# AolinFeng/PMP-VVC-TIP2023

Measured on AMD Instinct MI355X. Metric: CTUs/sec (luma QT+MTT inference+post-proc), higher is better.
Workload: dtype f16x3

## Files before the change

### include/pmp.h

```cpp
#ifndef PMP_H
#define PMP_H

#include <stdint.h>

#ifdef __cplusplus
extern "C" {
#endif

#define PMP_OK 0
#define PMP_E_INVALID (-1)
#define PMP_E_HIP (-2)
#define PMP_E_NOWEIGHTS (-3)
#define PMP_E_IO (-4)
#define PMP_E_NOMEM (-5)
#define PMP_E_NODEVICE (-6)
#define PMP_E_RANGE (-7)

enum { PMP_LUMA = 0, PMP_CHROMA = 1 };
enum { PMP_NET_LUMA_Q = 0, PMP_NET_LUMA_MSBD = 1, PMP_NET_CHROMA_Q = 2, PMP_NET_CHROMA_MSBD = 3 };

typedef struct pmp_ctx pmp_ctx;

typedef struct {
    const char *name;
// ... 143 lines not shown
} pmp_stem_shape;
int pmp_stem_forward_device(pmp_ctx *ctx, const pmp_stem_shape *shape, const float *d_x, const float *const d_w[3],
                            const float *const d_b[3], float *d_y);
int pmp_stem_backward_device(pmp_ctx *ctx, const pmp_stem_shape *shape, const float *d_x, const float *d_y, const float *const d_w[3],
                             const float *d_g_y, float *d_g_x , float *const d_g_w[3], float *const d_g_b[3]);

int pmp_infer_msbd(pmp_ctx *ctx, int comp, int qp, const uint8_t *block_y, const uint8_t *block_u, const uint8_t *block_v,
                   const float *qt_in, int64_t n, float *bt, float *dire);
int pmp_infer_msbd_device(pmp_ctx *ctx, int comp, int qp, const uint8_t *d_block_y, const uint8_t *d_block_u, const uint8_t *d_block_v,
                          const float *d_qt_in, int64_t n, float *d_bt, float *d_dire);

int pmp_read_depth_dump(const char *path, int frames, int height, int width, int is_chroma, uint8_t *qt8, uint8_t *bt16,
                        int8_t *dire16, int64_t *n_unknown);

int pmp_write_partition_file(const char *path, int frames, int height, int width, const uint8_t *hor,
                             const uint8_t *ver, const uint8_t *qt_u8, const int8_t *dire_i8);
int64_t pmp_format_partition_text(int frames, int height, int width, const uint8_t *hor, const uint8_t *ver,
                                  const uint8_t *qt_u8, const int8_t *dire_i8, char *buf, int64_t cap);

int64_t pmp_format_partition_rows(int width, int block_rows, const uint8_t *hor, const uint8_t *ver, const uint8_t *qt_u8,
                                  const int8_t *dire_i8, char *buf, int64_t cap, int64_t *row_section_bytes);
int64_t pmp_format_partition_rows_records(int width, int block_rows, const uint8_t *rec, char *buf, int64_t cap,
                                          int64_t *row_section_bytes);
int pmp_tile_partition_rows_records(int width, int block_rows, const uint8_t *rec, uint8_t *out_hor, uint8_t *out_ver, uint8_t *out_qt,
                                    int8_t *out_dire);

int pmp_write_partition_binary(const char *path, int frames, int height, int width, const uint8_t *hor, const uint8_t *ver,
                               const uint8_t *qt_u8, const int8_t *dire_i8);

int pmp_tile_partition_maps(int frames, int height, int width, const uint8_t *hor, const uint8_t *ver, const uint8_t *qt_u8,
                            const int8_t *dire_i8, uint8_t *out_hor, uint8_t *out_ver, uint8_t *out_qt, int8_t *out_dire);

int pmp_ktime_enable(pmp_ctx *ctx, uint32_t mask);
int pmp_ktime_classes(void);
const char *pmp_ktime_name(int cls);
int pmp_ktime_get(pmp_ctx *ctx, int cls, int64_t *launches, double *ms, double *flops);

int pmp_debug_set_conv_variant(int variant);

int pmp_debug_set_winograd(pmp_ctx *ctx, int on);

int pmp_debug_set_fusion(pmp_ctx *ctx, int on);

int pmp_debug_activation_report(pmp_ctx *ctx, int comp, int qp, int exps[5], float seg_amax[5], char *buf, int64_t cap);
int pmp_debug_set_activation_scales(pmp_ctx *ctx, int on);

int pmp_debug_set_taps(pmp_ctx *ctx, int on);
int64_t pmp_debug_get_tap(pmp_ctx *ctx, const char *name, double *out, int64_t cap, int dims[4], int *c_real);

int pmp_debug_poison_workspace(pmp_ctx *ctx, int pattern);

int64_t pmp_debug_pack_f16x3(const float *w, int cout, int cin, int k, uint16_t *out, int64_t cap, int *scale_exp);

int pmp_debug_read_weights_file(const char *path, int *net_id, int *qp, int *ntensors, int64_t *nfloats, double *checksum);

int pmp_debug_conv_bench(pmp_ctx *ctx, int n, int h, int w, int cin, int cout, int k, int iters, double *ms_f32,
                         double *ms_x6, double *max_abs_diff, double *max_abs_ref);

typedef struct pmp_rb_case {
    int n, h, w, cin, cout, k;
    int gate, pool, out_f32;
    int exp_x, exp_gate, exp_out;
} pmp_rb_case;
int pmp_debug_run_resblock(pmp_ctx *ctx, const pmp_rb_case *cs, const float *x, const float *w0, const float *w2, const float *wsc,
                           const float *gate, int *saturated, char *kernels, int64_t cap);

#ifdef __cplusplus
}
#endif
#endif
```

### pmp_vvc_tip2023_amd/_lib.py

```python
import ctypes as C
import os

_HERE = os.path.dirname(os.path.abspath(__file__))
LIB_PATH = os.path.join(_HERE, "libpmp_hip.so")
HOSTASAN_LIB_PATH = os.path.join(_HERE, "libpmp_hostasan.so")

PMP_LUMA, PMP_CHROMA = 0, 1
PMP_RECORD_BYTES = 1344
PMP_MSBT_LEAF_BUDGET = 4096
PMP_VAL_NSTATS = 20
PMP_LOSS_NTERMS = 13
PMP_MSBT_INCONSISTENT, PMP_MSBT_QT_DEEP, PMP_MSBT_BUDGET = 1, 2, 4
NET_IDS = {"Luma_Q": 0, "Luma_MSBD": 1, "Chroma_Q": 2, "Chroma_MSBD": 3}
ERRORS = {-1: "PMP_E_INVALID", -2: "PMP_E_HIP", -3: "PMP_E_NOWEIGHTS", -4: "PMP_E_IO", -5: "PMP_E_NOMEM", -6: "PMP_E_NODEVICE", -7: "PMP_E_RANGE"}


class PmpError(RuntimeError):
    def __init__(self, code, msg):
        super().__init__("%s (%d): %s" % (ERRORS.get(code, "PMP_E_?"), code, msg))
        self.code = code


class TensorDesc(C.Structure):
    _fields_ = [("name", C.c_char_p), ("ndim", C.c_int), ("shape", C.c_int * 4), ("offset", C.c_int64)]
# ... 77 lines not shown
    "pmp_postprocess_device": (_I, [_VP, _I, _VP, _VP, _VP, _I64, _VP, _VP, _VP, _VP]),
    "pmp_set_partition_params": (_I, [_VP, _I, C.POINTER(PartitionParams)]),
    "pmp_get_partition_params": (_I, [_VP, _I, C.POINTER(PartitionParams)]),
    "pmp_parse_partition_params": (_I, [C.c_char_p, C.POINTER(PartitionParams)]),
    "pmp_infer_postprocess": (_I, [_VP, _I, _I, _VP, _VP, _VP, _I64, _VP, _VP, _VP, _VP, _VP, _VP, _VP]),
    "pmp_infer_postprocess_device": (_I, [_VP, _I, _I, _VP, _VP, _VP, _I64, _VP, _VP, _VP, _VP, _VP, _VP, _VP]),
    "pmp_postprocess_records_device": (_I, [_VP, _I, _VP, _VP, _VP, _I64, _VP]),
    "pmp_infer_postprocess_records_device": (_I, [_VP, _I, _I, _VP, _VP, _VP, _I64, _VP]),
    "pmp_cut_blocks": (_I, [_VP, _VP, _VP, _VP, _I, _I, _I, _I, _VP, _VP, _VP]),
    "pmp_cut_blocks_device": (_I, [_VP, _VP, _VP, _VP, _I, _I, _I, _I, _VP, _VP, _VP]),
    "pmp_msbt_labels": (_I, [_VP, _I, _VP, _VP, _VP, _I64, _VP, _VP]),
    "pmp_msbt_labels_device": (_I, [_VP, _I, _VP, _VP, _VP, _I64, _VP, _VP]),
    "pmp_label_partition": (_I, [_VP, _I, _VP, _VP, _VP, _I64, _VP, _VP, _VP]),
    "pmp_label_partition_device": (_I, [_VP, _I, _VP, _VP, _VP, _I64, _VP, _VP, _VP]),
    "pmp_label_partition_records_device": (_I, [_VP, _I, _VP, _VP, _VP, _I64, _VP, _VP]),
    "pmp_val_stats": (_I, [_VP, _I, _VP, _VP, _VP, _VP, _VP, _VP, _I64, _VP]),
    "pmp_val_stats_device": (_I, [_VP, _I, _VP, _VP, _VP, _VP, _VP, _VP, _I64, _VP, _VP]),
    "pmp_parse_loss_params": (_I, [C.c_char_p, C.POINTER(LossParams)]),
    "pmp_train_loss": (_I, [_VP, _I, _I, C.POINTER(LossParams), _VP, _VP, _VP, _VP, _VP, _VP, _I64, _VP, _VP, _VP, _VP, _VP]),
    "pmp_train_loss_device": (_I, [_VP, _I, _I, C.POINTER(LossParams), _VP, _VP, _VP, _VP, _VP, _VP, _I64, _VP, _VP, _VP, _VP, _VP]),
    "pmp_resblock_forward": (_I, [_VP, C.POINTER(RbShape)] + [_VP] * 6),
    "pmp_resblock_forward_device": (_I, [_VP, C.POINTER(RbShape)] + [_VP] * 6),
    "pmp_resblock_backward": (_I, [_VP, C.POINTER(RbShape)] + [_VP] * 11),
    "pmp_resblock_backward_device": (_I, [_VP, C.POINTER(RbShape)] + [_VP] * 11),
    "pmp_trunk_saved_bytes": (_I64, [C.POINTER(TrunkShape)]),
    "pmp_trunk_forward_device": (_I, [_VP, C.POINTER(TrunkShape), _VP, _VP, _VP, _VP]),
    "pmp_trunk_backward_device": (_I, [_VP, C.POINTER(TrunkShape), _VP, _VP, _VP, _VP, _VP]),
    "pmp_trunk_unpack_device": (_I, [_VP, C.POINTER(TrunkShape), _VP, _I, _VP]),
    "pmp_stem_forward_device": (_I, [_VP, C.POINTER(StemShape), _VP, _VP, _VP, _VP]),
    "pmp_stem_backward_device": (_I, [_VP, C.POINTER(StemShape)] + [_VP] * 7),
    "pmp_infer_msbd": (_I, [_VP, _I, _I, _VP, _VP, _VP, _VP, _I64, _VP, _VP]),
    "pmp_infer_msbd_device": (_I, [_VP, _I, _I, _VP, _VP, _VP, _VP, _I64, _VP, _VP]),
    "pmp_read_depth_dump": (_I, [C.c_char_p, _I, _I, _I, _I, _VP, _VP, _VP, C.POINTER(_I64)]),
    "pmp_write_partition_file": (_I, [C.c_char_p, _I, _I, _I, _VP, _VP, _VP, _VP]),
    "pmp_write_partition_binary": (_I, [C.c_char_p, _I, _I, _I, _VP, _VP, _VP, _VP]),
    "pmp_tile_partition_maps": (_I, [_I, _I, _I, _VP, _VP, _VP, _VP, _VP, _VP, _VP, _VP]),
    "pmp_format_partition_text": (_I64, [_I, _I, _I, _VP, _VP, _VP, _VP, _VP, _I64]),
    "pmp_format_partition_rows": (_I64, [_I, _I, _VP, _VP, _VP, _VP, _VP, _I64, _VP]),
    "pmp_format_partition_rows_records": (_I64, [_I, _I, _VP, _VP, _I64, _VP]),
    "pmp_tile_partition_rows_records": (_I, [_I, _I, _VP, _VP, _VP, _VP, _VP]),
    "pmp_ktime_enable": (_I, [_VP, _U32]),
    "pmp_ktime_classes": (_I, []),
    "pmp_ktime_name": (C.c_char_p, [_I]),
    "pmp_ktime_get": (_I, [_VP, _I, C.POINTER(_I64), C.POINTER(C.c_double), C.POINTER(C.c_double)]),
    "pmp_debug_set_conv_variant": (_I, [_I]),
    "pmp_debug_set_winograd": (_I, [_VP, _I]),
    "pmp_debug_set_fusion": (_I, [_VP, _I]),
    "pmp_debug_set_activation_scales": (_I, [_VP, _I]),
    "pmp_debug_activation_report": (_I, [_VP, _I, _I, C.POINTER(_I), C.POINTER(C.c_float), C.c_char_p, _I64]),
    "pmp_debug_set_taps": (_I, [_VP, _I]),
    "pmp_debug_get_tap": (_I64, [_VP, C.c_char_p, _VP, _I64, C.POINTER(_I), C.POINTER(_I)]),
    "pmp_debug_poison_workspace": (_I, [_VP, _I]),
    "pmp_debug_pack_f16x3": (C.c_int64, [C.POINTER(C.c_float), _I, _I, _I, C.POINTER(C.c_uint16), C.c_int64, C.POINTER(C.c_int)]),
    "pmp_debug_conv_bench": (_I, [_VP, _I, _I, _I, _I, _I, _I, _I] + [C.POINTER(C.c_double)] * 4),
    "pmp_debug_run_resblock": (_I, [_VP, _VP] + [C.POINTER(C.c_float)] * 5 + [C.POINTER(_I), C.c_char_p, _I64]),
}

_lib = None


def open_library(path, subset=False):
    if not os.path.isfile(path):
        raise ImportError("%s is missing - build it with `make -C %s` (or __graft_entry__.build())"
                          % (path, os.path.join(_HERE, "csrc")))
    lib = C.CDLL(path)
    for name, (res, args) in SIGNATURES.items():
        if subset and not hasattr(lib, name):
            continue
        fn = getattr(lib, name)
        fn.restype = res
        fn.argtypes = args
    return lib


def _torch_first():
    import sys
    if "torch" not in sys.modules:
        try:
            import torch
        except ImportError:
            pass


def load(path=None):
    global _lib
    if _lib is None:
        _torch_first()
        _lib = open_library(path or LIB_PATH)
    elif path is not None and os.path.abspath(path) != os.path.abspath(_lib._name):
        raise RuntimeError("a different build of the library is already loaded: %s" % _lib._name)
    return _lib


def check(rc, ctx=None):
    if rc < 0:
        msg = load().pmp_last_error(ctx)
        raise PmpError(int(rc), msg.decode() if msg else "")
    return rc
```

### pmp_vvc_tip2023_amd/csrc/api_debug.cpp

```cpp
#include <algorithm>
#include <cmath>
#include <cstring>

#include "pmp_host.h"

namespace pmp {

KScope::KScope(pmp_ctx *c_, hipStream_t stream_, int cls_, double flops_) : c(c_), stream(stream_), cls(cls_), on(false), a(nullptr), b(nullptr), flops(flops_)
{
    on = (c->kmask >> cls) & 1u;
    if (on) { a = c->event_pool.get(); b = c->event_pool.get(); hipEventRecord(a, stream); }
}

KScope::~KScope()
{
    if (on) { hipEventRecord(b, stream); c->krec[cls].push_back(KTimeRec{a, b, flops}); }
}

void ktime_drain(pmp_ctx *c)
{
    for (int k = 0; k < K_NCLASS; ++k) {
        for (auto &r : c->krec[k]) {
            float ms = 0.f;
            hipEventSynchronize(r.b);
// ... 30 lines not shown
}

}

using namespace pmp;

extern "C" {

int pmp_debug_set_conv_variant(int variant)
{
    int rc;
    if (abl_set_conv_variant(variant, &rc)) return rc;
    if (variant != 2) return set_err(nullptr, PMP_E_INVALID, "pmp_debug_set_conv_variant: this library ships only the default form (2); the A/B and timing-only builds are in tools/abl/libpmp_hip_abl.so (make -C tools/abl)");
    return PMP_OK;
}

int pmp_debug_set_fusion(pmp_ctx *c, int on)
{
    CHECK_CTX(c);
    const int rc = settle(c);
    if (rc != PMP_OK) return rc;
    if (on < 0 || on > 3) return set_err(c, PMP_E_INVALID, "pmp_debug_set_fusion: 0 (none), 1 (all), 2 (16x16 tails only), 3 (32x32 ResidualBlocks only)");
    c->fuse16 = (on == 1 || on == 2) ? 1 : 0;
    c->fuse32 = (on == 1 || on == 3) ? 1 : 0;
    return PMP_OK;
}

int pmp_debug_set_winograd(pmp_ctx *c, int on)
{
    CHECK_CTX(c);
    int rc = settle(c);
    if (rc != PMP_OK) return rc;
    if (abl_set_winograd(c, on, &rc)) return rc;
    if (on) return set_err(c, PMP_E_INVALID, "pmp_debug_set_winograd: the Winograd-x form is built into tools/abl/libpmp_hip_abl.so only (make -C tools/abl)");
    return PMP_OK;
}

int pmp_debug_conv_bench(pmp_ctx *c, int n, int h, int w, int cin, int cout, int k, int iters, double *ms_f32, double *ms_x6,
                         double *max_abs_diff, double *max_abs_ref)
{
    CHECK_CTX(c);
    if (n <= 0 || (h & 15) || (w & 15) || (cin & 15) || (cout & 15) || cout > 64 || (k != 1 && k != 3 && k != 5) || iters <= 0)
        return set_err(c, PMP_E_INVALID, "pmp_debug_conv_bench: bad shape");
    const size_t nx = (size_t)n * cin * h * w, ny = (size_t)n * cout * h * w;
    std::vector<float> hx(nx), hw((size_t)cout * cin * k * k);
    unsigned long long st = 0x1234567ull;
    auto rnd = [&]() { st = st * 6364136223846793005ull + 1442695040888963407ull; return (float)((st >> 40) / 16777216.0) * 2.f - 1.f; };
    for (auto &v : hx) v = rnd() * 3.f;
    const float ws = 1.f / sqrtf((float)cin * k * k);
    for (auto &v : hw) v = rnd() * ws;
    std::vector<float> wp = pack_mfma(hw.data(), cout, cin, k, k, cout, cin);
    const bool h2 = c->precision == PMP_PRECISION_F16X3;
    const int kexp = h2_scale_exp(hw.data(), hw.size());
    std::vector<unsigned short> wx = h2 ? pack_h2(hw.data(), cout, cin, k, k, cout, cin, kexp) : pack_x6(hw.data(), cout, cin, k, k, cout, cin);
    AblBench ab;
    DevBuf bx, by, by2, bwp, bxs, bys, bwx;
    hipError_t e = hipSuccess;
    auto A = [&](DevBuf &b, size_t bytes) {
        if (e != hipSuccess) return;
        if ((e = hipMalloc(&b.p, bytes)) == hipSuccess) b.cap = bytes;
        else b.p = nullptr;
    };
    A(bx, nx * 4); A(by, ny * 4); A(by2, ny * 4); A(bwp, wp.size() * 4);
    A(bxs, nx * 6); A(bys, ny * 6); A(bwx, wx.size() * 2);
    int rc = PMP_OK;
    if (e != hipSuccess) rc = hip_fail(c, e, "hipMalloc(conv bench)");
    if (rc == PMP_OK) {
        float *dx = (float *)bx.p, *dy = (float *)by.p, *dy2 = (float *)by2.p, *dwp = (float *)bwp.p;
        unsigned short *dxs = (unsigned short *)bxs.p, *dys = (unsigned short *)bys.p, *dwx = (unsigned short *)bwx.p;
        hipMemcpy(dx, hx.data(), nx * 4, hipMemcpyHostToDevice);
        hipMemcpy(dwp, wp.data(), wp.size() * 4, hipMemcpyHostToDevice);
        hipMemcpy(dwx, wx.data(), wx.size() * 2, hipMemcpyHostToDevice);
        ConvMfmaArgs a{};
        a.x = dx; a.w = dwp; a.out = dy; a.N = n; a.H = h; a.W = w; a.Cin = cin; a.Cout = cout; a.KH = a.KW = k; a.relu = 1;
        ConvX6Args b{};
        b.x = dxs; b.x_stride = nx; b.w = dwx; b.out = dys; b.out_stride = ny;
        b.N = n; b.H = h; b.W = w; b.Cin = cin; b.Cout = cout; b.KH = b.KW = k; b.relu = 1;
        b.out_scale = std::ldexp(1.f, -kexp);
        abl_bench_prepare(c, ab, hw.data(), k, cin, cout, h2, b);
        auto launch_split = [&]() { return h2 ? launch_conv_h2(c->stream, b) : launch_conv_x6(c->stream, b); };
        hipEvent_t e0 = c->event_pool.get(), e1 = c->event_pool.get();
        if (h2) launch_f32_to_split2(c->stream, dx, dxs, nx, nx);
        else launch_f32_to_split3(c->stream, dx, dxs, nx, nx);
        launch_conv_mfma(c->stream, a);
        e = launch_split();
        float ms = 0.f;
        hipEventRecord(e0, c->stream);
        for (int i = 0; i < iters; ++i) launch_conv_mfma(c->stream, a);
        hipEventRecord(e1, c->stream); hipEventSynchronize(e1); hipEventElapsedTime(&ms, e0, e1);
        if (ms_f32) *ms_f32 = ms / iters;
        hipEventRecord(e0, c->stream);
        for (int i = 0; i < iters; ++i) launch_split();
        hipEventRecord(e1, c->stream); hipEventSynchronize(e1); hipEventElapsedTime(&ms, e0, e1);
        if (ms_x6) *ms_x6 = ms / iters;
        abl_bench_report(c, ab, h2, n, h, w, k, cout, b, launch_split);
        if (h2) launch_split2_to_f32(c->stream, dys, dy2, ny, ny);
        else launch_split3_to_f32(c->stream, dys, dy2, ny, ny);
        std::vector<float> y1(ny), y2(ny);
        hipMemcpyAsync(y1.data(), dy, ny * 4, hipMemcpyDeviceToHost, c->stream);
        hipMemcpyAsync(y2.data(), dy2, ny * 4, hipMemcpyDeviceToHost, c->stream);
        hipError_t es = hipStreamSynchronize(c->stream);
        if (e == hipSuccess) e = es;
        if (e == hipSuccess) e = hipGetLastError();
        double md = 0, mr = 0;
        for (size_t i = 0; i < ny; ++i) { md = fmax(md, fabs((double)y1[i] - y2[i])); mr = fmax(mr, fabs((double)y1[i])); }
        if (max_abs_diff) *max_abs_diff = md;
        if (max_abs_ref) *max_abs_ref = mr;
// ... 165 lines not shown
```

### pmp_vvc_tip2023_amd/csrc/conv_f16x3.hip

```cpp
#include <cstdio>
#include <type_traits>

#include "pmp_kernels.h"
#include "split3.h"

namespace pmp {

template <int KH, int KW, int NTHR = 256>
struct StagePlanH {
    unsigned off[GeoH<KH, KW, 16, NTHR>::NLD];
    unsigned valid;
};

template <int KH, int KW, int NTHR = 256>
__device__ __forceinline__ void h2_plan(StagePlanH<KH, KW, NTHR> &p, size_t plane_stride, int H, int W, int ty, int tx)
{
    typedef GeoH<KH, KW, 16, NTHR> G;
    constexpr int PY = KH / 2, PX = KW / 2;
    p.valid = 0;
#pragma unroll
    for (int k = 0; k < G::NLD; ++k) {
        const int i = min((int)threadIdx.x + k * NTHR, G::PIECES - 1);
        const int sp = i / G::PLANE, j = i - sp * G::PLANE, pix = j >> 1, half = j & 1;
        const int row = pix / G::TW, col = pix - row * G::TW;
// ... 211 lines not shown
                for (int m = 0; m < RW; ++m)
#pragma unroll
                    for (int nt = 0; nt < CW; ++nt) acc[m][nt] = __builtin_amdgcn_mfma_f32_16x16x32_f16(w0[nt], x0[m], acc[m][nt], 0, 0, 0);
                __builtin_amdgcn_sched_barrier(0);
                if (ks + 1 < NK) {
                    const char *pn = xaddr(ks + 1);
#pragma unroll
                    for (int m = 0; m < RW; ++m) x0[m] = *reinterpret_cast<const f16x8 *>(pn + m * G::TW * 32);
                }
                __builtin_amdgcn_sched_barrier(0);
#pragma unroll
                for (int m = 0; m < RW; ++m)
#pragma unroll
                    for (int nt = 0; nt < CW; ++nt) acc[m][nt] = __builtin_amdgcn_mfma_f32_16x16x32_f16(w0[nt], x1[m], acc[m][nt], 0, 0, 0);
                __builtin_amdgcn_sched_barrier(0);
                if (!W0DB) {
#pragma unroll
                    for (int nt = 0; nt < CW; ++nt) w0[nt] = wf[(0 * NT + nt) * 64];
                }
                __builtin_amdgcn_sched_barrier(0);
            }
            if (MODE == 1 && g < 2) {
                const char *pl = buf + O_LAST + pb;
#pragma unroll
                for (int m = 0; m < RW; ++m) {
                    x0[m] = *reinterpret_cast<const f16x8 *>(pl + m * G::TW * 32);
                    x1[m] = *reinterpret_cast<const f16x8 *>(pl + G::PLANE * 16 + m * G::TW * 32);
                }
            }
        }
        if (more) h2_stage_store<KH, KW, NTHR>(plan, lds + ((cb + 1) & 1) * G::BUF, rs, NK > LAG ? (NK - LAG) * PER : 0);
        __syncthreads();
    };

    typedef std::integral_constant<int, 0> M0;
    typedef std::integral_constant<int, 1> M1;
    typedef std::integral_constant<int, 2> M2;
    typedef std::integral_constant<int, 0> T0;
    typedef std::integral_constant<int, 1> T1;
    typedef std::integral_constant<int, 2> T2;
    if (paired) {
        for (int cb = 0; cb + 2 < CB; cb += 2) {
            group(M1{}, T0{}, cb);
            group(M2{}, T0{}, cb + 1);
        }
        group(M1{}, T1{}, CB - 2);
        group(M2{}, T2{}, CB - 1);
    } else {
        for (int cb = 0; cb + 1 < CB; ++cb) group(M0{}, T0{}, cb);
        group(M0{}, T2{}, CB - 1);
    }
}

template <int NT>
__device__ __forceinline__ void h2_epilogue(const ConvX6Args &a, f32x4 (&acc)[WaveTile<NT>::RW][WaveTile<NT>::CW], int n, int ty, int tx);

template <int NT>
__device__ __forceinline__ void h2_shortcut32(const ConvX6Args &a, int n, int ty, int tx, u32x4 *lds,
                                              f32x4 (&acc)[WaveTile<NT>::RW][WaveTile<NT>::CW])
{
    typedef WaveTile<NT> WT;
    constexpr int RW = WT::RW, CW = WT::CW;
    const int tid = threadIdx.x, lane = tid & 63, wave = tid >> 6, xl = lane & 15, g = lane >> 4;
    const int rh = wave % WT::RSPLIT, ch = wave / WT::RSPLIT;
    const int W = a.W;
    const size_t grp_sz = (size_t)a.H * W * 16;
    const unsigned short *base = a.x_sc + (size_t)n * 2 * grp_sz + ((size_t)(ty * 16) * W + tx * 16) * 16;
    __syncthreads();
    u32x4 r[8];
#pragma unroll
    for (int k = 0; k < 8; ++k) {
        const int i = tid + k * 256, grp = i >> 10, plane = (i >> 9) & 1, j = i & 511, px = j >> 1, half = j & 1;
        r[k] = *reinterpret_cast<const u32x4 *>(base + plane * a.sc_stride + grp * grp_sz + ((size_t)(px >> 4) * W + (px & 15)) * 16 + half * 8);
    }
    const f16x8 *wl = reinterpret_cast<const f16x8 *>(a.w_sc) + lane + ch * CW * 64;
    f16x8 w0[CW], w1[CW];
#pragma unroll
    for (int nt = 0; nt < CW; ++nt) { w0[nt] = wl[(0 * NT + nt) * 64]; w1[nt] = wl[(1 * NT + nt) * 64]; }
#pragma unroll
    for (int k = 0; k < 8; ++k) lds[tid + k * 256] = r[k];
    __syncthreads();
    const char *px = reinterpret_cast<const char *>(lds) + (g >> 1) * 16384 + ((rh * RW * 16 + xl) * 2 + (g & 1)) * 16;
#pragma unroll
    for (int h = 0; h < RW / 2; ++h) {
        f16x8 xa[2], xb[2];
#pragma unroll
        for (int m = 0; m < 2; ++m) {
            xa[m] = *reinterpret_cast<const f16x8 *>(px + (h * 2 + m) * 16 * 32);
            xb[m] = *reinterpret_cast<const f16x8 *>(px + 8192 + (h * 2 + m) * 16 * 32);
        }
#pragma unroll
        for (int m = 0; m < 2; ++m)
#pragma unroll
            for (int nt = 0; nt < CW; ++nt) acc[h * 2 + m][nt] = __builtin_amdgcn_mfma_f32_16x16x32_f16(w1[nt], xa[m], acc[h * 2 + m][nt], 0, 0, 0);
#pragma unroll
        for (int m = 0; m < 2; ++m)
#pragma unroll
            for (int nt = 0; nt < CW; ++nt) acc[h * 2 + m][nt] = __builtin_amdgcn_mfma_f32_16x16x32_f16(w0[nt], xa[m], acc[h * 2 + m][nt], 0, 0, 0);
#pragma unroll
        for (int m = 0; m < 2; ++m)
#pragma unroll
            for (int nt = 0; nt < CW; ++nt) acc[h * 2 + m][nt] = __builtin_amdgcn_mfma_f32_16x16x32_f16(w0[nt], xb[m], acc[h * 2 + m][nt], 0, 0, 0);
    }
}

template <int KH, int KW, int NT, int SC, bool LEAN = false>
__global__ __launch_bounds__(256, NT == 4 && !LEAN ? 2 : 3) void conv_h2_kernel(ConvX6Args a)
{
    typedef GeoH<KH, KW> G;
    __shared__ u32x4 lds[2 * G::BUF];
    const int tiles_x = a.W >> 4, tiles = tiles_x * (a.H >> 4);
    int bid = blockIdx.x;
    if ((gridDim.x & 7) == 0) bid = (bid & 7) * (gridDim.x >> 3) + (bid >> 3);
    const int n = bid / tiles, t = bid - n * tiles, ty = t / tiles_x, tx = t - ty * tiles_x;
    typedef WaveTile<NT> WT;
    constexpr int RW = WT::RW, CW = WT::CW;

    f32x4 acc[RW][CW];
#pragma unroll
    for (int m = 0; m < RW; ++m)
#pragma unroll
        for (int nt = 0; nt < CW; ++nt) acc[m][nt] = (f32x4){0.f, 0.f, 0.f, 0.f};

    h2_accumulate<KH, KW, NT, LEAN>(a.x, a.x_stride, a.w, a.Cin, a.H, a.W, n, ty, tx, lds, acc);
    if (SC == 2) h2_shortcut32<NT>(a, n, ty, tx, lds, acc);
    else if (SC) h2_accumulate<1, 1, NT, LEAN>(a.x_sc, a.sc_stride, a.w_sc, a.Csc, a.H, a.W, n, ty, tx, lds, acc);
    h2_epilogue<NT>(a, acc, n, ty, tx);
}

template <int NT>
__device__ __forceinline__ void h2_epilogue(const ConvX6Args &a, f32x4 (&acc)[WaveTile<NT>::RW][WaveTile<NT>::CW], int n, int ty, int tx)
{
    typedef WaveTile<NT> WT;
    constexpr int RW = WT::RW, CW = WT::CW;
    int tid = threadIdx.x;
    asm volatile("" : "+v"(tid));
    const int lane = tid & 63, wave = tid >> 6, xl = lane & 15, g = lane >> 4;
    const int rh = wave % WT::RSPLIT, ch = wave / WT::RSPLIT;
    const int H = a.H, W = a.W;
    const size_t grp = (size_t)H * W * 16;

    const float inv_scale = a.out_scale;
    const unsigned off0 = (unsigned)(((size_t)n * NT + ch * CW) * grp + ((size_t)(ty * 16 + rh * RW) * W + tx * 16 + xl) * 16 + g * 4);
    const unsigned row_el = (unsigned)W * 16;
    const unsigned off0w = off0 - (unsigned)(g * 4) + (unsigned)(8 * (g >> 1)) + (unsigned)(g & 1) * row_el;
    u32x4 ra[RW / 2][CW], rbv[RW / 2][CW];
    auto res_load = [&](int nt, int slot) __attribute__((always_inline)) {
#pragma unroll
        for (int m = 0; m < RW; m += 2) {
            const unsigned off = off0w + (unsigned)m * row_el + (unsigned)nt * (unsigned)grp;
            ra[m >> 1][slot] = __builtin_nontemporal_load(reinterpret_cast<const u32x4 *>(a.res + off));
            rbv[m >> 1][slot] = __builtin_nontemporal_load(reinterpret_cast<const u32x4 *>(a.res + off + a.res_stride));
        }
    };
    auto res_add = [&](int nt, int slot) __attribute__((always_inline)) {
#pragma unroll
        for (int m = 0; m < RW; m += 2) {
            u32x4 p = ra[m >> 1][slot], q = rbv[m >> 1][slot];
            rows16_swap(p);
            rows16_swap(q);
            acc[m][nt] = acc[m][nt] * inv_scale + h2_sum4_lo(p, q);
            acc[m + 1][nt] = acc[m + 1][nt] * inv_scale + h2_sum4_hi(p, q);
        }
    };
    if (a.res) {
#pragma unroll
        for (int nt = 0; nt < CW; ++nt) res_load(nt, nt);
#pragma unroll
        for (int nt = 0; nt < CW; ++nt) res_add(nt, nt);
    } else {
#pragma unroll
        for (int nt = 0; nt < CW; ++nt)
#pragma unroll
            for (int m = 0; m < RW; ++m) acc[m][nt] = acc[m][nt] * inv_scale;
    }
    float amax = 0.f;
#pragma unroll
    for (int nt = 0; nt < CW; ++nt) {
#pragma unroll
        for (int m = 0; m < RW; ++m) {
            const unsigned off = off0 + (unsigned)m * row_el + (unsigned)nt * (unsigned)grp;
            f32x4 v = acc[m][nt];
            if (a.relu) { v.x = fmaxf(v.x, 0.f); v.y = fmaxf(v.y, 0.f); v.z = fmaxf(v.z, 0.f); v.w = fmaxf(v.w, 0.f); }
            if (a.gate) v *= load_split2_4(a.gate + off, a.gate_stride);
            amax = sat_amax4(amax, v);
            acc[m][nt] = v;
// ... 126 lines not shown
```

### pmp_vvc_tip2023_amd/csrc/pack.cpp

```cpp
#include <algorithm>
#include <cmath>
#include <cstring>
#include <utility>

#include "pmp_hostonly.h"

namespace pmp {

std::vector<float> pack_mfma(const float *w, int cout, int cin, int kh, int kw, int cout_pad, int cin_pad)
{
    const int taps = kh * kw, CB = cin_pad / 16, NT = cout_pad / 16;
    std::vector<float> out((size_t)CB * taps * NT * 64 * 4, 0.f);
    for (int cb = 0; cb < CB; ++cb)
        for (int t = 0; t < taps; ++t)
            for (int nt = 0; nt < NT; ++nt)
                for (int l = 0; l < 64; ++l)
                    for (int j = 0; j < 4; ++j) {
                        const int co = nt * 16 + (l & 15), ci = cb * 16 + 4 * (l >> 4) + j;
                        float v = 0.f;
                        if (co < cout && ci < cin) v = w[((size_t)co * cin + ci) * taps + t];
                        out[((((size_t)cb * taps + t) * NT + nt) * 64 + l) * 4 + j] = v;
                    }
    return out;
}
// ... 72 lines not shown
                    const float r1 = v - bf16_f32(h0);
                    const unsigned short h1 = bf16_rne(r1);
                    const float r2 = r1 - bf16_f32(h1);
                    const unsigned short h2 = bf16_rne(r2);
                    const unsigned short hs[3] = {h0, h1, h2};
                    for (int sp = 0; sp < 3; ++sp) out[(((st * 3 + sp) * NT + nt) * 64 + l) * 8 + j] = hs[sp];
                }
    return out;
}

int h2_scale_exp(const float *w, size_t n)
{
    float m = 0.f;
    for (size_t i = 0; i < n; ++i) m = std::fmax(m, std::fabs(w[i]));
    if (!(m > 0.f) || !std::isfinite(m)) return 0;
    int e = 0;
    std::frexp(m, &e);
    int k = 13 - e;
    return k < -100 ? -100 : (k > 24 ? 24 : k);
}

std::vector<unsigned short> pack_h2(const float *w, int cout, int cin, int kh, int kw, int cout_pad, int cin_pad, int scale_exp)
{
    const int taps = kh * kw, CB = cin_pad / 16, NT = cout_pad / 16;
    const bool paired = (CB % 2 == 0) && (taps % 2 == 1);
    const float S = std::ldexp(1.f, scale_exp);
    struct Half { int cb, tap; };
    std::vector<std::pair<Half, Half>> steps;
    if (paired) {
        for (int cb = 0; cb < CB; ++cb) {
            if (cb & 1) steps.push_back({{cb - 1, taps - 1}, {cb, taps - 1}});
            for (int ks = 0; ks < (taps - 1) / 2; ++ks) steps.push_back({{cb, 2 * ks}, {cb, 2 * ks + 1}});
        }
    } else {
        for (int cb = 0; cb < CB; ++cb)
            for (int ks = 0; ks < (taps + 1) / 2; ++ks) steps.push_back({{cb, 2 * ks}, {cb, 2 * ks + 1}});
    }
    std::vector<unsigned short> out(steps.size() * 2 * NT * 64 * 8, 0);
    for (size_t st = 0; st < steps.size(); ++st)
        for (int nt = 0; nt < NT; ++nt) {
            unsigned short *o0 = out.data() + ((st * 2 + 0) * NT + nt) * 512, *o1 = out.data() + ((st * 2 + 1) * NT + nt) * 512;
            for (int l = 0; l < 64; ++l) {
                const int g = l >> 4;
                const Half h = (g >> 1) ? steps[st].second : steps[st].first;
                const int co = nt * 16 + (l & 15), ci0 = h.cb * 16 + 8 * (g & 1), t = h.tap;
                float v[8];
                for (int j = 0; j < 8; ++j) v[j] = (co < cout && ci0 + j < cin && t < taps) ? w[((size_t)co * cin + ci0 + j) * taps + t] * S : 0.f;
                split8(v, o0 + l * 8, o1 + l * 8);
            }
        }
    return out;
}

std::vector<unsigned short> pack_stem_h2(const float *w32, int cin, int k1, int scale_exp)
{
    const int RPS = k1 > 8 ? 3 : 5, KPP = (k1 + RPS - 1) / RPS, KS = cin * KPP;
    const float S = std::ldexp(1.f, scale_exp);
    std::vector<unsigned short> out((size_t)KS * 3 * 2 * 64 * 8, 0);
    for (int ks = 0; ks < KS; ++ks)
        for (int nt = 0; nt < 2; ++nt)
            for (int l = 0; l < 64; ++l) {
                const int g = l >> 4, co = nt * 16 + (l & 15), ci = ks / KPP, r0 = (ks % KPP) * RPS;
                float v[8];
                for (int j = 0; j < 8; ++j) {
                    const int kk = 8 * g + j, dyl = kk / k1, dx = kk % k1, dy = r0 + dyl;
                    v[j] = (dyl < RPS && dy < k1) ? w32[(((size_t)co * cin + ci) * k1 + dy) * k1 + dx] * S : 0.f;
                }
                unsigned short *o0 = out.data() + ((((size_t)ks * 3 + 0) * 2 + nt) * 64 + l) * 8, *o1 = o0 + 2 * 64 * 8, *o2 = o1 + 2 * 64 * 8;
                split8(v, o0, o1);
                float r[8];
                unsigned short dummy[8];
                for (int j = 0; j < 8; ++j) {
                    _Float16 h0, h1;
                    std::memcpy(&h0, o0 + j, 2); std::memcpy(&h1, o1 + j, 2);
                    r[j] = (v[j] - (float)h0) - (float)h1;
                }
                split8(r, o2, dummy);
            }
    return out;
}

std::vector<float> pack_plain(const float *w, int cout, int cin, int kh, int kw)
{
    const int taps = kh * kw;
    std::vector<float> out((size_t)taps * cin * cout);
    for (int t = 0; t < taps; ++t)
        for (int ci = 0; ci < cin; ++ci)
            for (int co = 0; co < cout; ++co) out[((size_t)t * cin + ci) * cout + co] = w[((size_t)co * cin + ci) * taps + t];
    return out;
}

}

using namespace pmp;
#define set_err(ctx_unused, code, msg) set_err_global((code), (msg))

extern "C" {

int64_t pmp_debug_pack_f16x3(const float *w, int cout, int cin, int k, uint16_t *out, int64_t cap, int *scale_exp)
{
    if (!w || cout <= 0 || cin <= 0 || (k != 1 && k != 3 && k != 5) || !scale_exp)
        return set_err(nullptr, PMP_E_INVALID, "pmp_debug_pack_f16x3: bad arguments");
    const int kexp = h2_scale_exp(w, (size_t)cout * cin * k * k);
    *scale_exp = kexp;
    const std::vector<unsigned short> v = pack_h2(w, cout, cin, k, k, (cout + 15) & ~15, (cin + 15) & ~15, kexp);
    if (out && (int64_t)v.size() <= cap) memcpy(out, v.data(), v.size() * sizeof(unsigned short));
    return (int64_t)v.size();
}

}
```

### pmp_vvc_tip2023_amd/csrc/pmp_hostonly.h

```cpp
#pragma once
#include <stdint.h>

#include <string>
#include <vector>

#include "../../include/pmp.h"

namespace pmp {

int set_err_global(int code, const std::string &msg);
const char *global_err();

std::vector<float> pack_mfma(const float *w, int cout, int cin, int kh, int kw, int cout_pad, int cin_pad);
std::vector<unsigned short> pack_x6(const float *w, int cout, int cin, int kh, int kw, int cout_pad, int cin_pad);
std::vector<unsigned short> pack_h2(const float *w, int cout, int cin, int kh, int kw, int cout_pad, int cin_pad, int scale_exp);
int h2_scale_exp(const float *w, size_t n);
void h2_split8(const float *v, unsigned short *h0, unsigned short *h1);
std::vector<unsigned short> pack_stem_h2(const float *w32, int cin, int k1, int scale_exp);
std::vector<float> pack_plain(const float *w, int cout, int cin, int kh, int kw);


struct WeightTensor { std::string name; int ndim = 0; int shape[4] = {0, 0, 0, 0}; long long offset = 0; };
struct WeightFile { std::string net; int qp = -1; std::vector<WeightTensor> tensors; std::vector<float> payload;
                    std::vector<int> act_exp;
                    bool have_fp = false; uint64_t act_mtt_fp = 0, act_qt_fp = 0; };
int read_pmpw(const char *path, WeightFile &wf);
constexpr int PMP_ACT_EXP_MAX = 30;
constexpr int PMP_ACT_EXP_ATT_MAX = 6;
uint64_t fingerprint_tensors(const float *blob, const pmp_tensor_desc *descs, int ndesc);
int net_id_of(const std::string &net);

bool partition_params_valid(const pmp_partition_params &p, std::string &why);

}
```

### pmp_vvc_tip2023_amd/csrc/weights_pack.cpp

```cpp
#include <algorithm>
#include <cmath>
#include <cstring>
#include <utility>

#include "pmp_host.h"

namespace pmp {

namespace {

struct Blob {
    const float *blob;
    const pmp_tensor_desc *descs;
    int ndesc;
    const pmp_tensor_desc *find(const std::string &name) const
    {
        for (int i = 0; i < ndesc; ++i)
            if (descs[i].name && name == descs[i].name) return &descs[i];
        return nullptr;
    }
};

int roundup16(int v) { return (v + 15) & ~15; }

// ... 27 lines not shown
        fixups.clear();
        stage.clear();
        return PMP_OK;
    }
};

}

namespace {

int need(pmp_ctx *c, const Blob &b, const std::string &name, std::initializer_list<int> shape, const float **out)
{
    const pmp_tensor_desc *d = b.find(name);
    if (!d) return set_err(c, PMP_E_INVALID, "weights: missing tensor " + name);
    if (d->ndim != (int)shape.size()) return set_err(c, PMP_E_INVALID, "weights: wrong rank for " + name);
    int i = 0;
    for (int s : shape)
        if (d->shape[i++] != s) return set_err(c, PMP_E_INVALID, "weights: wrong shape for " + name);
    *out = b.blob + d->offset;
    return PMP_OK;
}

int load_rb(pmp_ctx *c, const Blob &b, Uploader &up, const std::string &name, int cin, int cout, int k, bool direct, unsigned mask)
{
    RBWeights &r = up.nw->rb[name];
    r.cin = cin; r.cout = cout; r.k = k; r.direct = direct; r.has_sc = cin != cout;
    r.cin_pad = roundup16(cin); r.cout_pad = roundup16(cout);
    const float *w0, *w2, *wsc = nullptr;
    int rc;
    if ((rc = need(c, b, name + ".left.0.weight", {cout, cin, k, k}, &w0))) return rc;
    if ((rc = need(c, b, name + ".left.2.weight", {cout, cout, k, k}, &w2))) return rc;
    if (cin != cout && (rc = need(c, b, name + ".shortcut.0.weight", {cout, cin, 1, 1}, &wsc))) return rc;
    if (direct) {
        if (!r.w0) {
            if ((rc = up.upload(pack_plain(w0, cout, cin, k, k), &r.w0))) return rc;
            if ((rc = up.upload(pack_plain(w2, cout, cout, k, k), &r.w2))) return rc;
            if (wsc && (rc = up.upload(pack_plain(wsc, cout, cin, 1, 1), &r.wsc))) return rc;
        }
    } else {
        if ((mask & (1u << PMP_PRECISION_F32)) && !r.w0) {
            if ((rc = up.upload(pack_mfma(w0, cout, cin, k, k, r.cout_pad, r.cin_pad), &r.w0))) return rc;
            if ((rc = up.upload(pack_mfma(w2, cout, cout, k, k, r.cout_pad, r.cout_pad), &r.w2))) return rc;
            if (wsc && (rc = up.upload(pack_mfma(wsc, cout, cin, 1, 1, r.cout_pad, r.cin_pad), &r.wsc))) return rc;
        }
        if ((mask & (1u << PMP_PRECISION_BF16X6)) && !r.w0x) {
            if ((rc = up.upload16(pack_x6(w0, cout, cin, k, k, r.cout_pad, r.cin_pad), &r.w0x))) return rc;
            if ((rc = up.upload16(pack_x6(w2, cout, cout, k, k, r.cout_pad, r.cout_pad), &r.w2x))) return rc;
            if (wsc && (rc = up.upload16(pack_x6(wsc, cout, cin, 1, 1, r.cout_pad, r.cin_pad), &r.wscx))) return rc;
        }
        if ((mask & (1u << PMP_PRECISION_F16X3)) && !r.w0h) {
            r.k0 = h2_scale_exp(w0, (size_t)cout * cin * k * k);
            r.k2 = h2_scale_exp(w2, (size_t)cout * cout * k * k);
            if (wsc) r.k2 = std::min(r.k2, h2_scale_exp(wsc, (size_t)cout * cin));
            if ((rc = up.upload16(pack_h2(w0, cout, cin, k, k, r.cout_pad, r.cin_pad, r.k0), &r.w0h))) return rc;
            if ((rc = up.upload16(pack_h2(w2, cout, cout, k, k, r.cout_pad, r.cout_pad, r.k2), &r.w2h))) return rc;
            if (wsc && (rc = up.upload16(pack_h2(wsc, cout, cin, 1, 1, r.cout_pad, r.cin_pad, r.k2), &r.wsch))) return rc;
        }
        if ((rc = abl_pack_rb(w0, w2, k, cin, cout, mask, r, [&](const std::vector<unsigned short> &v, unsigned short **dst) { return up.upload16(v, dst); }))) return rc;
    }
    return PMP_OK;
}

int load_head(pmp_ctx *c, const Blob &b, Uploader &up, const std::string &name, int cout, int slot)
{
    const float *w, *bias;
    int rc;
    if ((rc = need(c, b, name + ".weight", {cout, 8, 3, 3}, &w))) return rc;
    if ((rc = need(c, b, name + ".bias", {cout}, &bias))) return rc;
    if (up.nw->head_w[slot]) return PMP_OK;
    if ((rc = up.upload(pack_plain(w, cout, 8, 3, 3), &up.nw->head_w[slot]))) return rc;
    return up.upload(std::vector<float>(bias, bias + cout), &up.nw->head_b[slot]);
}

}

int load_single_rb(pmp_ctx *c, NetWeights &nw, int cin, int cout, int k, const float *w0, const float *w2, const float *wsc, unsigned mask)
{
    std::vector<float> blob(w0, w0 + (size_t)cout * cin * k * k);
    blob.insert(blob.end(), w2, w2 + (size_t)cout * cout * k * k);
    if (cin != cout) blob.insert(blob.end(), wsc, wsc + (size_t)cout * cin);
    const pmp_tensor_desc descs[3] = {{"rb.left.0.weight", 4, {cout, cin, k, k}, 0},
                                      {"rb.left.2.weight", 4, {cout, cout, k, k}, (int64_t)cout * cin * k * k},
                                      {"rb.shortcut.0.weight", 4, {cout, cin, 1, 1}, (int64_t)cout * cin * k * k + (int64_t)cout * cout * k * k}};
    Uploader up{c, &nw};
    int rc = load_rb(c, Blob{blob.data(), descs, cin != cout ? 3 : 2}, up, "rb", cin, cout, k, false, mask);
    if (rc != PMP_OK) { up.abandon(); return rc; }
    return up.finalize();
}

void free_net_weights(NetWeights &w)
{
    for (void *p : w.allocs) hipFree(p);
    w = NetWeights();
}

static int build_net(pmp_ctx *c, int net_id, const Blob &b, NetWeights &nw, unsigned mask)
{
    const bool luma = net_id == PMP_NET_LUMA_Q || net_id == PMP_NET_LUMA_MSBD;
    const bool msbd = net_id == PMP_NET_LUMA_MSBD || net_id == PMP_NET_CHROMA_MSBD;
    Uploader up{c, &nw};
    int rc = PMP_OK;
    const bool want_h2 = mask & (1u << PMP_PRECISION_F16X3);
    auto fail = [&](int code) { up.abandon(); return code; };

    if (!msbd) {
        const int cin = luma ? 1 : 3, k1 = luma ? 9 : 5, kq = luma ? 5 : 3;
        const float *w, *bias;
        if ((rc = need(c, b, "conv_q1.weight", {32, cin, k1, k1}, &w))) return fail(rc);
// ... 158 lines not shown
```

Measured before the change: 15240.

## Add sliding-window 5x5 f16x3 conv kernel with pass-paired weight packing

Adds a specialised 5x5, 64-output-channel f16x3 convolution path. Each wave slides down 20 input rows and reuses every loaded input vector across the five kernel rows, issuing MFMAs into 16 row accumulators. Weights are repacked so each pass pairs two kx taps, or the kx=4 taps of two channel blocks, with next-pass weights prefetched and the next channel group's global-to-LDS staging spread across the MFMA stream. In exchange the kernel is much more complex, uses a different accumulator tile shape and launch bound, and needs a matching host-side weight packer.

```diff
diff --git a/include/pmp.h b/include/pmp.h
--- a/include/pmp.h
+++ b/include/pmp.h
@@ -219,6 +219,8 @@
 
 int64_t pmp_debug_pack_f16x3(const float *w, int cout, int cin, int k, uint16_t *out, int64_t cap, int *scale_exp);
 
+int64_t pmp_debug_pack_f16x3_slide5(const float *w, int cout, int cin, int scale_exp, uint16_t *out, int64_t cap);
+
 int pmp_debug_read_weights_file(const char *path, int *net_id, int *qp, int *ntensors, int64_t *nfloats, double *checksum);
 
 int pmp_debug_conv_bench(pmp_ctx *ctx, int n, int h, int w, int cin, int cout, int k, int iters, double *ms_f32,
diff --git a/pmp_vvc_tip2023_amd/_lib.py b/pmp_vvc_tip2023_amd/_lib.py
--- a/pmp_vvc_tip2023_amd/_lib.py
+++ b/pmp_vvc_tip2023_amd/_lib.py
@@ -153,6 +153,7 @@
     "pmp_debug_get_tap": (_I64, [_VP, C.c_char_p, _VP, _I64, C.POINTER(_I), C.POINTER(_I)]),
     "pmp_debug_poison_workspace": (_I, [_VP, _I]),
     "pmp_debug_pack_f16x3": (C.c_int64, [C.POINTER(C.c_float), _I, _I, _I, C.POINTER(C.c_uint16), C.c_int64, C.POINTER(C.c_int)]),
+    "pmp_debug_pack_f16x3_slide5": (C.c_int64, [C.POINTER(C.c_float), _I, _I, _I, C.POINTER(C.c_uint16), C.c_int64]),
     "pmp_debug_conv_bench": (_I, [_VP, _I, _I, _I, _I, _I, _I, _I] + [C.POINTER(C.c_double)] * 4),
     "pmp_debug_run_resblock": (_I, [_VP, _VP] + [C.POINTER(C.c_float)] * 5 + [C.POINTER(_I), C.c_char_p, _I64]),
 }
@@ -187,7 +188,7 @@
     global _lib
     if _lib is None:
         _torch_first()
-        _lib = open_library(path or LIB_PATH)
+        _lib = open_library(path or LIB_PATH, subset=path is not None and os.path.abspath(path) != os.path.abspath(LIB_PATH))
     elif path is not None and os.path.abspath(path) != os.path.abspath(_lib._name):
         raise RuntimeError("a different build of the library is already loaded: %s" % _lib._name)
     return _lib
diff --git a/pmp_vvc_tip2023_amd/csrc/api_debug.cpp b/pmp_vvc_tip2023_amd/csrc/api_debug.cpp
--- a/pmp_vvc_tip2023_amd/csrc/api_debug.cpp
+++ b/pmp_vvc_tip2023_amd/csrc/api_debug.cpp
@@ -106,7 +106,7 @@
     std::vector<float> wp = pack_mfma(hw.data(), cout, cin, k, k, cout, cin);
     const bool h2 = c->precision == PMP_PRECISION_F16X3;
     const int kexp = h2_scale_exp(hw.data(), hw.size());
-    std::vector<unsigned short> wx = h2 ? pack_h2(hw.data(), cout, cin, k, k, cout, cin, kexp) : pack_x6(hw.data(), cout, cin, k, k, cout, cin);
+    std::vector<unsigned short> wx = h2 ? pack_h2_conv(hw.data(), cout, cin, k, k, cout, cin, kexp, 0) : pack_x6(hw.data(), cout, cin, k, k, cout, cin);
     AblBench ab;
     DevBuf bx, by, by2, bwp, bxs, bys, bwx;
     hipError_t e = hipSuccess;
diff --git a/pmp_vvc_tip2023_amd/csrc/conv_f16x3.hip b/pmp_vvc_tip2023_amd/csrc/conv_f16x3.hip
--- a/pmp_vvc_tip2023_amd/csrc/conv_f16x3.hip
+++ b/pmp_vvc_tip2023_amd/csrc/conv_f16x3.hip
@@ -287,14 +287,136 @@
     }
 }
 
-template <int NT>
-__device__ __forceinline__ void h2_epilogue(const ConvX6Args &a, f32x4 (&acc)[WaveTile<NT>::RW][WaveTile<NT>::CW], int n, int ty, int tx);
-
-template <int NT>
+template <int LD0, int LDS_, int ST0, int STS_, bool FETCH_>
+struct SlideSched {
+    static constexpr int ld0 = LD0, lds = LDS_, st0 = ST0, sts = STS_;
+    static constexpr bool FETCH = FETCH_;
+};
+
+__device__ __forceinline__ void h2_slide5(const unsigned short *__restrict__ x, size_t plane_stride, const unsigned short *__restrict__ wpk,
+                                          int C, int H, int W, int n, int ty, int tx, u32x4 *lds, f32x4 (&acc)[16][1])
+{
+    constexpr int NTHR = 256;
+    typedef GeoH<5, 5, 16, NTHR> G;
+    const int lane = threadIdx.x & 63, wave = threadIdx.x >> 6, xl = lane & 15, g = lane >> 4;
+    const int CB = C >> 4;
+    const size_t grp_sz = (size_t)H * W * 16;
+    const unsigned short *grp0 = x + (size_t)n * CB * grp_sz;
+    constexpr int PASS = 5 * 2 * 4 * 64;
+    const int last = (CB >> 1) * 5 + (CB & 1) * 3 - 1;
+    const f16x8 *wl = reinterpret_cast<const f16x8 *>(wpk) + lane + wave * 64;
+    f16x8 w0[5], w1[5], w0n[5], w1n[5];
+    u32x4 r[G::NLD];
+    StagePlanH<5, 5, NTHR> plan;
+    h2_plan<5, 5, NTHR>(plan, plane_stride, H, W, ty, tx);
+#pragma unroll
+    for (int ky = 0; ky < 5; ++ky) { w0[ky] = wl[(ky * 2 + 0) * 256]; w1[ky] = wl[(ky * 2 + 1) * 256]; }
+    __syncthreads();
+    h2_stage_load<5, 5, NTHR>(plan, grp0, r);
+    h2_stage_store<5, 5, NTHR>(plan, lds, r);
+    __syncthreads();
+    const int pb = (xl * 2 + (g & 1)) * 16 + (g >> 1) * 32;
+    int stream = 0;
+
+    auto pass = [&](auto t0_tag, auto sched_tag, const char *px, const unsigned short *nxt_grp, u32x4 *dst) __attribute__((always_inline)) {
+        constexpr int T0 = decltype(t0_tag)::value;
+        typedef decltype(sched_tag) S;
+        ++stream;
+        const f16x8 *wf = wl + (size_t)min(stream, last) * PASS;
+        f16x8 xa[2], xb[2];
+        xa[0] = *reinterpret_cast<const f16x8 *>(px);
+        xb[0] = *reinterpret_cast<const f16x8 *>(px + G::PLANE * 16);
+#pragma unroll
+        for (int rr = 0; rr < 20; ++rr) {
+            if (rr + 1 < 20) {
+                xa[(rr + 1) & 1] = *reinterpret_cast<const f16x8 *>(px + (rr + 1) * G::TW * 32);
+                xb[(rr + 1) & 1] = *reinterpret_cast<const f16x8 *>(px + G::PLANE * 16 + (rr + 1) * G::TW * 32);
+            }
+            __builtin_amdgcn_sched_barrier(0);
+            if (rr == 0) {
+#pragma unroll
+                for (int ky = 0; ky < 5; ++ky) { w1n[ky] = wf[(ky * 2 + 1) * 256]; w0n[ky] = wf[(ky * 2 + 0) * 256]; }
+            }
+            if (S::FETCH) {
+#pragma unroll
+                for (int k = 0; k < G::NLD; ++k) {
+                    if (T0 + rr == S::ld0 + S::lds * k) h2_stage_load<5, 5, NTHR>(plan, nxt_grp, r, k, k + 1);
+                    if (T0 + rr == S::st0 + S::sts * k) h2_stage_store<5, 5, NTHR>(plan, dst, r, k, k + 1);
+                }
+            }
+            __builtin_amdgcn_sched_barrier(0);
+#pragma unroll
+            for (int ky = 0; ky < 5; ++ky)
+                if (rr - ky >= 0 && rr - ky < 16) acc[rr - ky][0] = __builtin_amdgcn_mfma_f32_16x16x32_f16(w1[ky], xa[rr & 1], acc[rr - ky][0], 0, 0, 0);
+#pragma unroll
+            for (int ky = 0; ky < 5; ++ky)
+                if (rr - ky >= 0 && rr - ky < 16) acc[rr - ky][0] = __builtin_amdgcn_mfma_f32_16x16x32_f16(w0[ky], xa[rr & 1], acc[rr - ky][0], 0, 0, 0);
+#pragma unroll
+            for (int ky = 0; ky < 5; ++ky)
+                if (rr - ky >= 0 && rr - ky < 16) acc[rr - ky][0] = __builtin_amdgcn_mfma_f32_16x16x32_f16(w0[ky], xb[rr & 1], acc[rr - ky][0], 0, 0, 0);
+            __builtin_amdgcn_sched_barrier(0);
+        }
+#pragma unroll
+        for (int ky = 0; ky < 5; ++ky) { w0[ky] = w0n[ky]; w1[ky] = w1n[ky]; }
+    };
+
+    typedef std::integral_constant<int, 0> R0;
+    typedef std::integral_constant<int, 20> R20;
+    typedef std::integral_constant<int, 40> R40;
+    typedef SlideSched<1, 4, 14, 4, true> SEven;
+    typedef SlideSched<1, 3, 22, 3, true> SOdd;
+    typedef SlideSched<0, 0, 0, 0, false> SNone;
+    static_assert(SEven::st0 + SEven::sts * (G::NLD - 1) < 40 && SOdd::st0 >= 20 && SOdd::st0 + SOdd::sts * (G::NLD - 1) < 60, "every slice is stored inside its group");
+
+    auto even = [&](int cb) __attribute__((always_inline)) {
+        const char *buf = reinterpret_cast<const char *>(lds + (cb & 1) * G::BUF);
+        u32x4 *dst = lds + ((cb + 1) & 1) * G::BUF;
+        const unsigned short *nxt = grp0 + (size_t)(cb + 1) * grp_sz;
+        pass(R0{}, SEven{}, buf + pb, nxt, dst);
+        pass(R20{}, SEven{}, buf + 2 * 32 + pb, nxt, dst);
+        __syncthreads();
+    };
+    auto odd = [&](auto sched_tag, int cb) __attribute__((always_inline)) {
+        const char *buf = reinterpret_cast<const char *>(lds + (cb & 1) * G::BUF);
+        const char *part = reinterpret_cast<const char *>(lds + ((cb + 1) & 1) * G::BUF);
+        u32x4 *dst = lds + ((cb + 1) & 1) * G::BUF;
+        const unsigned short *nxt = grp0 + (size_t)min(cb + 1, CB - 1) * grp_sz;
+        pass(R0{}, sched_tag, (g < 2 ? part : buf) + 4 * 32 + (xl * 2 + (g & 1)) * 16, nxt, dst);
+        h2_lds_barrier();
+        pass(R20{}, sched_tag, buf + pb, nxt, dst);
+        pass(R40{}, sched_tag, buf + 2 * 32 + pb, nxt, dst);
+        __syncthreads();
+    };
+    int cb = 0;
+    for (; cb + 2 < CB; cb += 2) {
+        even(cb);
+        odd(SOdd{}, cb + 1);
+    }
+    if (CB & 1) {
+        const char *buf = reinterpret_cast<const char *>(lds + (cb & 1) * G::BUF);
+        pass(R0{}, SNone{}, buf + pb, grp0, lds);
+        pass(R20{}, SNone{}, buf + 2 * 32 + pb, grp0, lds);
+        pass(R40{}, SNone{}, buf + 4 * 32 + (xl * 2 + (g & 1)) * 16, grp0, lds);
+        __syncthreads();
+    } else {
+        even(cb);
+        odd(SNone{}, cb + 1);
+    }
+}
+
+template <int KH, int KW, int NT, int SC>
+struct H2Tile {
+    static constexpr bool SLIDE = KH == 5 && KW == 5 && NT == 4 && SC != 1;
+    typedef WaveTile<NT, SLIDE ? 2 : 0> WT;
+};
+
+template <int NT, class WT>
+__device__ __forceinline__ void h2_epilogue(const ConvX6Args &a, f32x4 (&acc)[WT::RW][WT::CW], int n, int ty, int tx);
+
+template <int NT, class WT>
 __device__ __forceinline__ void h2_shortcut32(const ConvX6Args &a, int n, int ty, int tx, u32x4 *lds,
-                                              f32x4 (&acc)[WaveTile<NT>::RW][WaveTile<NT>::CW])
-{
-    typedef WaveTile<NT> WT;
+                                              f32x4 (&acc)[WT::RW][WT::CW])
+{
     constexpr int RW = WT::RW, CW = WT::CW;
     const int tid = threadIdx.x, lane = tid & 63, wave = tid >> 6, xl = lane & 15, g = lane >> 4;
     const int rh = wave % WT::RSPLIT, ch = wave / WT::RSPLIT;
@@ -340,7 +462,7 @@
 }
 
 template <int KH, int KW, int NT, int SC, bool LEAN = false>
-__global__ __launch_bounds__(256, NT == 4 && !LEAN ? 2 : 3) void conv_h2_kernel(ConvX6Args a)
+__global__ __launch_bounds__(256, NT == 4 && (!LEAN || H2Tile<KH, KW, NT, SC>::SLIDE) ? 2 : 3) void conv_h2_kernel(ConvX6Args a)
 {
     typedef GeoH<KH, KW> G;
     __shared__ u32x4 lds[2 * G::BUF];
@@ -348,7 +470,7 @@
     int bid = blockIdx.x;
     if ((gridDim.x & 7) == 0) bid = (bid & 7) * (gridDim.x >> 3) + (bid >> 3);
     const int n = bid / tiles, t = bid - n * tiles, ty = t / tiles_x, tx = t - ty * tiles_x;
-    typedef WaveTile<NT> WT;
+    typedef typename H2Tile<KH, KW, NT, SC>::WT WT;
     constexpr int RW = WT::RW, CW = WT::CW;
 
     f32x4 acc[RW][CW];
@@ -357,16 +479,20 @@
 #pragma unroll
         for (int nt = 0; nt < CW; ++nt) acc[m][nt] = (f32x4){0.f, 0.f, 0.f, 0.f};
 
-    h2_accumulate<KH, KW, NT, LEAN>(a.x, a.x_stride, a.w, a.Cin, a.H, a.W, n, ty, tx, lds, acc);
-    if (SC == 2) h2_shortcut32<NT>(a, n, ty, tx, lds, acc);
-    else if (SC) h2_accumulate<1, 1, NT, LEAN>(a.x_sc, a.sc_stride, a.w_sc, a.Csc, a.H, a.W, n, ty, tx, lds, acc);
-    h2_epilogue<NT>(a, acc, n, ty, tx);
-}
-
-template <int NT>
-__device__ __forceinline__ void h2_epilogue(const ConvX6Args &a, f32x4 (&acc)[WaveTile<NT>::RW][WaveTile<NT>::CW], int n, int ty, int tx)
-{
-    typedef WaveTile<NT> WT;
+    if constexpr (H2Tile<KH, KW, NT, SC>::SLIDE) {
+        h2_slide5(a.x, a.x_stride, a.w, a.Cin, a.H, a.W, n, ty, tx, lds, acc);
+        if (SC == 2) h2_shortcut32<NT, WT>(a, n, ty, tx, lds, acc);
+    } else {
+        h2_accumulate<KH, KW, NT, LEAN>(a.x, a.x_stride, a.w, a.Cin, a.H, a.W, n, ty, tx, lds, acc);
+        if (SC == 2) h2_shortcut32<NT, WT>(a, n, ty, tx, lds, acc);
+        else if (SC) h2_accumulate<1, 1, NT, LEAN>(a.x_sc, a.sc_stride, a.w_sc, a.Csc, a.H, a.W, n, ty, tx, lds, acc);
+    }
+    h2_epilogue<NT, WT>(a, acc, n, ty, tx);
+}
+
+template <int NT, class WT>
+__device__ __forceinline__ void h2_epilogue(const ConvX6Args &a, f32x4 (&acc)[WT::RW][WT::CW], int n, int ty, int tx)
+{
     constexpr int RW = WT::RW, CW = WT::CW;
     int tid = threadIdx.x;
     asm volatile("" : "+v"(tid));
diff --git a/pmp_vvc_tip2023_amd/csrc/pack.cpp b/pmp_vvc_tip2023_amd/csrc/pack.cpp
--- a/pmp_vvc_tip2023_amd/csrc/pack.cpp
+++ b/pmp_vvc_tip2023_amd/csrc/pack.cpp
@@ -148,6 +148,47 @@
     return out;
 }
 
+std::vector<unsigned short> pack_h2_slide5(const float *w, int cout, int cin, int cin_pad, int scale_exp)
+{
+    const int CB = cin_pad / 16, NT = 4, taps = 25;
+    const float S = std::ldexp(1.f, scale_exp);
+    struct Half { int cb, kx; };
+    std::vector<std::pair<Half, Half>> passes;
+    for (int p = 0; p + 1 < CB; p += 2) {
+        passes.push_back({{p, 0}, {p, 1}});
+        passes.push_back({{p, 2}, {p, 3}});
+        passes.push_back({{p, 4}, {p + 1, 4}});
+        passes.push_back({{p + 1, 0}, {p + 1, 1}});
+        passes.push_back({{p + 1, 2}, {p + 1, 3}});
+    }
+    if (CB & 1) {
+        passes.push_back({{CB - 1, 0}, {CB - 1, 1}});
+        passes.push_back({{CB - 1, 2}, {CB - 1, 3}});
+        passes.push_back({{CB - 1, 4}, {-1, 0}});
+    }
+    std::vector<unsigned short> out(passes.size() * 5 * 2 * NT * 512, 0);
+    for (size_t ps = 0; ps < passes.size(); ++ps)
+        for (int ky = 0; ky < 5; ++ky)
+            for (int nt = 0; nt < NT; ++nt) {
+                unsigned short *o0 = out.data() + (((ps * 5 + ky) * 2 + 0) * NT + nt) * 512, *o1 = o0 + NT * 512;
+                for (int l = 0; l < 64; ++l) {
+                    const int g = l >> 4;
+                    const Half h = (g >> 1) ? passes[ps].second : passes[ps].first;
+                    const int co = nt * 16 + (l & 15), ci0 = h.cb * 16 + 8 * (g & 1), t = ky * 5 + h.kx;
+                    float v[8];
+                    for (int j = 0; j < 8; ++j) v[j] = (h.cb >= 0 && co < cout && ci0 + j < cin) ? w[((size_t)co * cin + ci0 + j) * taps + t] * S : 0.f;
+                    split8(v, o0 + l * 8, o1 + l * 8);
+                }
+            }
+    return out;
+}
+
+std::vector<unsigned short> pack_h2_conv(const float *w, int cout, int cin, int kh, int kw, int cout_pad, int cin_pad, int scale_exp, int csc_pad)
+{
+    if (PMP_H2_SLIDE5 && kh == 5 && kw == 5 && cout_pad == 64 && (csc_pad == 0 || csc_pad == 32)) return pack_h2_slide5(w, cout, cin, cin_pad, scale_exp);
+    return pack_h2(w, cout, cin, kh, kw, cout_pad, cin_pad, scale_exp);
+}
+
 std::vector<unsigned short> pack_stem_h2(const float *w32, int cin, int k1, int scale_exp)
 {
     const int RPS = k1 > 8 ? 3 : 5, KPP = (k1 + RPS - 1) / RPS, KS = cin * KPP;
@@ -204,4 +245,12 @@
     return (int64_t)v.size();
 }
 
-}
+int64_t pmp_debug_pack_f16x3_slide5(const float *w, int cout, int cin, int scale_exp, uint16_t *out, int64_t cap)
+{
+    if (!w || cout <= 0 || cout > 64 || cin <= 0) return set_err(nullptr, PMP_E_INVALID, "pmp_debug_pack_f16x3_slide5: bad arguments");
+    const std::vector<unsigned short> v = pack_h2_slide5(w, cout, cin, (cin + 15) & ~15, scale_exp);
+    if (out && (int64_t)v.size() <= cap) memcpy(out, v.data(), v.size() * sizeof(unsigned short));
+    return (int64_t)v.size();
+}
+
+}
diff --git a/pmp_vvc_tip2023_amd/csrc/pmp_hostonly.h b/pmp_vvc_tip2023_amd/csrc/pmp_hostonly.h
--- a/pmp_vvc_tip2023_amd/csrc/pmp_hostonly.h
+++ b/pmp_vvc_tip2023_amd/csrc/pmp_hostonly.h
@@ -14,6 +14,11 @@
 std::vector<float> pack_mfma(const float *w, int cout, int cin, int kh, int kw, int cout_pad, int cin_pad);
 std::vector<unsigned short> pack_x6(const float *w, int cout, int cin, int kh, int kw, int cout_pad, int cin_pad);
 std::vector<unsigned short> pack_h2(const float *w, int cout, int cin, int kh, int kw, int cout_pad, int cin_pad, int scale_exp);
+#ifndef PMP_H2_SLIDE5
+#define PMP_H2_SLIDE5 1
+#endif
+std::vector<unsigned short> pack_h2_slide5(const float *w, int cout, int cin, int cin_pad, int scale_exp);
+std::vector<unsigned short> pack_h2_conv(const float *w, int cout, int cin, int kh, int kw, int cout_pad, int cin_pad, int scale_exp, int csc_pad);
 int h2_scale_exp(const float *w, size_t n);
 void h2_split8(const float *v, unsigned short *h0, unsigned short *h1);
 std::vector<unsigned short> pack_stem_h2(const float *w32, int cin, int k1, int scale_exp);
diff --git a/pmp_vvc_tip2023_amd/csrc/weights_pack.cpp b/pmp_vvc_tip2023_amd/csrc/weights_pack.cpp
--- a/pmp_vvc_tip2023_amd/csrc/weights_pack.cpp
+++ b/pmp_vvc_tip2023_amd/csrc/weights_pack.cpp
@@ -103,8 +103,8 @@
             r.k0 = h2_scale_exp(w0, (size_t)cout * cin * k * k);
             r.k2 = h2_scale_exp(w2, (size_t)cout * cout * k * k);
             if (wsc) r.k2 = std::min(r.k2, h2_scale_exp(wsc, (size_t)cout * cin));
-            if ((rc = up.upload16(pack_h2(w0, cout, cin, k, k, r.cout_pad, r.cin_pad, r.k0), &r.w0h))) return rc;
-            if ((rc = up.upload16(pack_h2(w2, cout, cout, k, k, r.cout_pad, r.cout_pad, r.k2), &r.w2h))) return rc;
+            if ((rc = up.upload16(pack_h2_conv(w0, cout, cin, k, k, r.cout_pad, r.cin_pad, r.k0, 0), &r.w0h))) return rc;
+            if ((rc = up.upload16(pack_h2_conv(w2, cout, cout, k, k, r.cout_pad, r.cout_pad, r.k2, wsc ? r.cin_pad : 0), &r.w2h))) return rc;
             if (wsc && (rc = up.upload16(pack_h2(wsc, cout, cin, 1, 1, r.cout_pad, r.cin_pad, r.k2), &r.wsch))) return rc;
         }
         if ((rc = abl_pack_rb(w0, w2, k, cin, cout, mask, r, [&](const std::vector<unsigned short> &v, unsigned short **dst) { return up.upload16(v, dst); }))) return rc;
```

After: 15370 (median of 6 runs). About the same (+0.9%).
